# PriviligedLearningDistributedAerial/imitation

Measured on AMD Instinct MI355X. Metric: env-steps/sec (whole node) + final eval return, GAIL HalfCheetah-v4 at 1/2/4/8 MI355X, higher is better.
Workload: dtype mixed (fp32 master weights and accumulation; PPO products as split-bf16 x3 ~fp32, discriminator bf16); 1 GPU; model=GAIL: FeedForward32Policy[32,32]+RunningNorm / BasicRewardNet(32,32)+RunningNorm, global_batch=4096, seq_len=512, parallelism=dp1, engine=device, env=HalfCheetah-v4

## Files before the change

csrc/kernels/rollout.hip:

```cpp
#include <hip/hip_runtime.h>

#include "ia/engine.h"
#include "ia/envs.h"
#include "ia/wave.h"
#include "launchers.h"

namespace ia {
namespace {

constexpr int kNoiseFloats = 4096;

template <bool SPLIT>
struct Actor {
  static constexpr int KH = SPLIT ? 16 : 1;
  float w[kWaveMaxLayers][KH];
  const lf* wt[kWaveMaxLayers];
  float bias[kWaveMaxLayers];
  int k0[kWaveMaxLayers];
  int ng[kWaveMaxLayers];
  int dout[kWaveMaxLayers];
  int n_layers, hidden_act;
};

__host__ __device__ __forceinline__ int split_kh(int din) { return ((din + 1) / 2 + 3) & ~3; }
constexpr int kFullGroups = 16;
__host__ __device__ __forceinline__ int full_lds_floats(const WaveMLP& m) { return m.n_layers * 4 * kFullGroups * 64; }

__device__ __forceinline__ void nb_lane(int l, int lane, int& kh, int& ub) {
  const int r = lane >> 4;
  kh = (l & 1) ? (r >> 1) : (r & 1);
  ub = (l & 1) ? (r & 1) : (r >> 1);
}

template <bool SPLIT, bool NB = false>
__device__ void load_actor(const WaveMLP& m, Actor<SPLIT>& r, lf* wlds) {
  const int lane = threadIdx.x;
  r.n_layers = m.n_layers;
  r.hidden_act = m.hidden_act;
#pragma unroll
  for (int l = 0; l < kWaveMaxLayers; ++l) {
    int h = SPLIT ? (lane >> 5) : 0;
    int j = SPLIT ? (lane & 31) : lane;
    if (NB) {
      int ub;
      nb_lane(l, lane, h, ub);
      j = 16 * ub + (lane & 15);
    }
    const bool on = l < m.n_layers;
    const int din = on ? m.dims[l] : 0, dout = on ? m.dims[l + 1] : 0;
    const int kh = SPLIT ? split_kh(din) : 4 * kFullGroups;
    const int k0 = h ? kh : 0;
    r.k0[l] = k0;
    r.ng[l] = kh >> 2;
    r.dout[l] = dout;
    if (SPLIT) {
      const int kend = h ? din : kh;
#pragma unroll
      for (int i = 0; i < Actor<SPLIT>::KH; ++i) {
        const int k = k0 + i;
        r.w[l][i] = (on && j < dout && k < kend && k < din) ? m.W[l][j * din + k] : 0.f;
      }
    } else {
      r.wt[l] = wlds;
      if (on) {
        for (int k = 0; k < kh; ++k) wlds[((k >> 2) * 64 + lane) * 4 + (k & 3)] = (j < dout && k < din) ? m.W[l][j * din + k] : 0.f;
        wlds += kh * 64;
      }
    }
    r.bias[l] = (on && j < dout && h == 0) ? m.b[l][j] : 0.f;
  }
}

template <int HACT>
__device__ __forceinline__ float hidden_act(int act, float x) {
  if (HACT == ACT_TANH) return act_fast(ACT_TANH, x);
  if (HACT == ACT_RELU) return fmaxf(x, 0.f);
  return act_fast(act, x);
}

template <typename T>
__device__ __forceinline__ T pin(T x) {
  asm volatile("" : "+v"(x));
  return x;
}

template <bool SPLIT, int HACT, int NLT = -1, int HW = -1>
__device__ __forceinline__ float actor_forward(const Actor<SPLIT>& r, lf* xb) {
  const int lane = threadIdx.x;
  const int j = SPLIT ? (lane & 31) : lane;
  const lf4* x4 = (const lf4*)xb;
  float h = 0.f;
  const int nl = NLT > 0 ? NLT : r.n_layers;
#pragma unroll
  for (int l = 0; l < kWaveMaxLayers; ++l) {
    if (l < nl) {
      const lf4* src = x4 + (r.k0[l] >> 2);
      float acc0 = r.bias[l], acc1 = 0.f;
      if (SPLIT) {
#pragma unroll
        for (int g = 0; g < 4; ++g) {
          const f32v4 v = src[g];
          acc0 = fmaf(r.w[l][4 * g + 0], v.x, acc0);
          acc1 = fmaf(r.w[l][4 * g + 1], v.y, acc1);
          acc0 = fmaf(r.w[l][4 * g + 2], v.z, acc0);
          acc1 = fmaf(r.w[l][4 * g + 3], v.w, acc1);
        }
      } else {
        const lf4* w4 = (const lf4*)r.wt[l] + lane;
        float acc2 = 0.f, acc3 = 0.f;
#pragma unroll
        for (int g = 0; g < kFullGroups; ++g) {
          const f32v4 v = src[g], w = w4[g * 64];
          acc0 = fmaf(w.x, v.x, acc0);
          acc1 = fmaf(w.y, v.y, acc1);
          acc2 = fmaf(w.z, v.z, acc2);
          acc3 = fmaf(w.w, v.w, acc3);
        }
        acc0 += acc2;
        acc1 += acc3;
      }
      float acc = acc0 + acc1;
      if (SPLIT) acc = add_halves(acc);
      const bool last = l == nl - 1;
      const bool full = HW > 0 && !last;
      h = (full || j < r.dout[l]) ? (last ? acc : hidden_act<HACT>(r.hidden_act, acc)) : 0.f;
      if (!last) {
        wave_sync();
        if (SPLIT && HW <= 0) {
          if (lane < 32) xb[lane] = h;
        } else {
          xb[lane] = h;
        }
        wave_sync();
      }
    }
  }
  return h;
}

template <int I>
__device__ __forceinline__ float fmac_row_bcast(float acc, float x, float w) {
  if constexpr (I == 0)
    asm("s_nop 1\n\tv_fmac_f32_dpp %0, %1, %2 row_newbcast:%3 row_mask:0xf bank_mask:0xf"
        : "+v"(acc) : "v"(x), "v"(w), "i"(I));
  else
    asm("v_fmac_f32_dpp %0, %1, %2 row_newbcast:%3 row_mask:0xf bank_mask:0xf" : "+v"(acc) : "v"(x), "v"(w), "i"(I));
  return acc;
}

template <int I>
__device__ __forceinline__ void nb_dot(const float* w, float x, float& a0, float& a1) {
  if constexpr (I < 16) {
    a0 = fmac_row_bcast<I>(a0, x, w[I]);
    a1 = fmac_row_bcast<I + 1>(a1, x, w[I + 1]);
    nb_dot<I + 2>(w, x, a0, a1);
  }
}

template <int HACT, int NLT>
__device__ __forceinline__ float actor_forward_nb(const Actor<true>& r, float x) {
  static_assert(NLT > 0, "the row form needs the layer count at compile time");
#pragma unroll
  for (int l = 0; l < NLT; ++l) {
    float acc0 = r.bias[l], acc1 = 0.f;
    nb_dot<0>(r.w[l], x, acc0, acc1);
    const float acc = (l & 1) ? add_halves(acc0 + acc1) : add_rows16(acc0 + acc1);
    x = l == NLT - 1 ? acc : hidden_act<HACT>(r.hidden_act, acc);
  }
  return x;
}

__device__ __forceinline__ int actor_obs_index(int lane, int obs_dim) {
  return ((lane >> 4) & 1 ? split_kh(obs_dim) : 0) + (lane & 15);
}

__device__ __forceinline__ float env_step_lane0(const EnvParams& P, float* s, const float* action, int* term, uint64_t* rng) {
  return env_step(P, s, action, term, *rng);
}
__device__ __forceinline__ void env_reset_lane0(const EnvParams& P, float* s, float* o, uint64_t* rng) {
  env_reset(P, s, *rng);
  env_obs(P, s, o);
}

enum ChainEnv : int { CE_GENERIC = 0, CE_LOCO = 1, CE_LOCO3 = 2  };

struct LocoRegs {
  float q, qd;
  float rq[8], rv[8];
  float gear, stiff, damp, thrust, pcoup;
  float dt, drag, fwd_weight, healthy, ctrl_cost, inv_nj, inv_dt_total;
};

__device__ void loco_load(const LocoParams& p, const lf* s, LocoRegs& L) {
  const int lane = threadIdx.x, nq = loco_nq(p);
  const bool jl = lane < p.nj;
  L.q = jl ? s[p.nq_root + lane] : 0.f;
  L.qd = jl ? s[nq + p.nv_root + lane] : 0.f;
#pragma unroll
  for (int i = 0; i < 8; ++i) {
    L.rq[i] = i < p.nq_root ? s[i] : 0.f;
    L.rv[i] = i < p.nv_root ? s[nq + i] : 0.f;
  }
}

__device__ void loco_store(const LocoParams& p, const LocoRegs& L, lf* s) {
  const int lane = threadIdx.x, nq = loco_nq(p);
  if (lane < p.nj) {
    s[p.nq_root + lane] = L.q;
    s[nq + p.nv_root + lane] = L.qd;
  }
  if (lane == 0) {
#pragma unroll
    for (int i = 0; i < 8; ++i) {
      if (i < p.nq_root) s[i] = L.rq[i];
      if (i < p.nv_root) s[nq + i] = L.rv[i];
    }
  }
}

template <int ENV>
__device__ float loco_obs(const LocoParams& p, const LocoRegs& L, lf* sb, int oxi, float& ox) {
  const int lane = threadIdx.x;
  const int nr = ENV == CE_LOCO3 ? 3 : 8;
  const int nqr = ENV == CE_LOCO3 ? 3 : p.nq_root, nvr = ENV == CE_LOCO3 ? 3 : p.nv_root;
  const int npr = nqr - p.obs_skip, nj = p.nj;
  float rqi = 0.f, rvi = 0.f;
#pragma unroll
  for (int i = 0; i < nr; ++i) {
    rqi = (lane + p.obs_skip) == i ? L.rq[i] : rqi;
    rvi = lane == i ? L.rv[i] : rvi;
  }
  wave_sync();
  if (lane < npr) sb[lane] = rqi;
  if (lane < nj) {
    sb[npr + lane] = L.q;
    sb[npr + nj + nvr + lane] = L.qd;
  }
  if (lane < nvr) sb[npr + nj + lane] = rvi;
  wave_sync();
  const int D = npr + nj + nvr + nj;
  ox = sb[oxi];
  return lane < D ? sb[lane] : 0.f;
}

template <int ENV, int FS = -1>
__device__ float loco_step_regs(const LocoParams& p, LocoRegs& L, float a_in) {
  const int lane = threadIdx.x;
  const bool jl = lane < p.nj;
  const float a = jl ? fminf(fmaxf(a_in, -1.f), 1.f) : 0.f;
  const float ctrl = sum_lanes8(a * a);
  const float pitch = sum_lanes8(L.pcoup * a);
  const float x_before = L.rq[0];
  const float dt = L.dt;
  float q = L.q, qd = L.qd;
  const auto substep = [&]() {
    const float qdd = L.gear * a - L.stiff * q - L.damp * qd - 2.0f * __sinf(q);
    const float st_all = stance(q);
    const float st = jl ? st_all : 0.f;
    const float th_j = L.thrust * st * fmaxf(-qd, 0.f);
    qd = qd + dt * qdd;
    const float thrust = sum_lanes8(th_j);
    const float lift = sum_lanes8(st);
    const float vx = L.rv[0];
    L.rv[0] = vx + dt * (thrust - L.drag * vx * (1.0f + fabsf(vx)));
    if (ENV == CE_LOCO3) {
      L.rv[1] = L.rv[1] + dt * (-20.f * L.rq[1] - 4.f * L.rv[1] + 0.5f * (lift * L.inv_nj - 0.5f));
      L.rv[2] = L.rv[2] + dt * (-15.f * __sinf(L.rq[2]) - 3.f * L.rv[2] + pitch);
      L.rq[0] += dt * L.rv[0];
      L.rq[1] += dt * L.rv[1] * 1.f;
      L.rq[2] += dt * L.rv[2] * 1.f;
    } else {
      if (p.nv_root > 1) L.rv[1] = L.rv[1] + dt * (-20.f * L.rq[1] - 4.f * L.rv[1] + 0.5f * (lift * L.inv_nj - 0.5f));
      if (p.nv_root > 2) L.rv[2] = L.rv[2] + dt * (-15.f * __sinf(L.rq[2]) - 3.f * L.rv[2] + pitch);
#pragma unroll
      for (int i = 3; i < 8; ++i)
        if (i < p.nv_root) L.rv[i] = L.rv[i] * (1.f - 2.f * dt) + dt * 0.1f * pitch;
      L.rq[0] += dt * L.rv[0];
#pragma unroll
      for (int i = 1; i < 8; ++i) {
        if (i < p.nq_root) {
          if (i < p.nv_root) {
            L.rq[i] += dt * L.rv[i] * 1.f;
          } else {
            const int vi = i % p.nv_root;
            float v = 0.f;
#pragma unroll
            for (int u = 0; u < 8; ++u) v = u == vi ? L.rv[u] : v;
            L.rq[i] += dt * v * 0.1f;
          }
        }
      }
    }
    const float qn = q + dt * qd;
    const bool hi = qn > 1.2f, lo = qn < -1.2f;
    qd = (hi && qd > 0.f) || (lo && qd < 0.f) ? 0.f : qd;
    q = fminf(fmaxf(qn, -1.2f), 1.2f);
  };
  if constexpr (FS > 0) {
#pragma unroll
    for (int sub = 0; sub < FS; ++sub) substep();
  } else {
    for (int sub = 0; sub < p.frame_skip; ++sub) substep();
  }
  L.q = jl ? q : 0.f;
  L.qd = jl ? qd : 0.f;
  return L.fwd_weight * (L.rq[0] - x_before) * L.inv_dt_total + L.healthy - L.ctrl_cost * ctrl;
}

typedef __attribute__((address_space(1))) float gfl;
struct Cursors {
  gfl* obs;
  gfl* next_obs;
  gfl* act_raw;
  gfl* act_env;
  gfl* sc;
  int vec_step, act_step, sc_step;
};

__device__ __forceinline__ long long stamp(float dep) {
  long long t;
  asm volatile("s_memtime %0\n\ts_waitcnt lgkmcnt(0)" : "=s"(t) : "v"(dep));
  return t;
}

template <bool SPLIT, int ENV, int HACT, int NLT = -1, int HW = -1, int FS = -1, bool PROF = false, bool ROW = true>
__global__ __launch_bounds__(64) void rollout_chain_kernel(RolloutArgs a) {
  extern __shared__ __attribute__((aligned(16))) float lds_raw[];
  lf* xb = (lf*)lds_raw;
  lf* sb = xb + 64;
  lf* st = sb + 64;
  lf* act = st + kMaxState;
  lf* noise = act + 64;
  li* explore = (li*)(noise + kNoiseFloats);
  lf* wlds = (lf*)(explore + ((a.T + 3) & ~3));
  const int n = blockIdx.x;
  const int lane = threadIdx.x;
  const EnvParams& P = a.P;
  const int D = P.obs_dim;
  constexpr bool loco = ENV != CE_GENERIC;
  const bool discrete = !loco && a.n_actions > 0;
  const int A = discrete ? 1 : P.act_dim;
  const int AW = discrete ? a.n_actions : P.act_dim;
  const int S = state_size(P);

  constexpr bool NB = ROW && SPLIT && HW == 32 && NLT > 0;
  Actor<SPLIT> ar;
  load_actor<SPLIT, NB>(a.pi, ar, wlds);
  const int oxi = NB ? actor_obs_index(lane, D) : lane;
  const bool ox_on = oxi < D;
  const int oxr = ox_on ? oxi : lane - 64;
  const float nmean = pin((a.pi.norm_mean && ox_on) ? a.pi.norm_mean[oxi] : 0.f);
  const float nrstd = pin((a.pi.norm_mean && ox_on) ? rsqrtf(a.pi.norm_var[oxi] + a.pi.norm_eps) : 1.f);
  const float lstd = (!discrete && a.log_std && lane < A) ? a.log_std[lane] : 0.f;
  const float sd = pin(expf(lstd));
  const float lo = pin((!discrete && a.act_low && lane < A) ? a.act_low[lane] : 0.f);
  const float hi = pin((!discrete && a.act_high && lane < A) ? a.act_high[lane] : 0.f);

  for (int i = lane; i < S; i += 64) st[i] = a.state[(size_t)n * S + i];
  xb[lane] = 0.f;
  LocoRegs L{};
  if (loco) {
    const LocoParams& p = P.loco;
    const bool jl = lane < p.nj;
    L.gear = pin(jl ? p.gear[lane] : 0.f);
    L.stiff = pin(jl ? p.stiff[lane] : 0.f);
    L.damp = pin(jl ? p.damp[lane] : 0.f);
    L.thrust = pin(jl ? p.thrust[lane] : 0.f);
    L.pcoup = pin(jl ? p.pitch_coupling[lane] : 0.f);
    L.dt = pin(p.dt);
    L.drag = pin(p.drag);
    L.fwd_weight = pin(p.fwd_weight);
    L.healthy = pin(p.healthy_reward);
    L.ctrl_cost = pin(p.ctrl_cost);
    L.inv_nj = pin(1.f / (float)p.nj);
    L.inv_dt_total = pin(1.f / (p.dt * (float)p.frame_skip));
  }
  wave_sync();
  if (loco) loco_load(P.loco, st, L);

  Cursors c;
  c.vec_step = a.N * D;
  c.act_step = a.N * A;
  c.sc_step = a.N;
  c.obs = pin((gfl*)(a.obs_buf + (size_t)n * D + (lane < D ? lane : 0)));
  c.next_obs = pin((gfl*)(a.next_obs + (size_t)n * D + (lane < D ? lane : 0)));
  c.act_raw = pin((gfl*)(a.act_raw + (size_t)n * A + (lane < A ? lane : 0)));
  c.act_env = pin((gfl*)(a.act_env + (size_t)n * A + (lane < A ? lane : 0)));
  {
    float* b = lane == 0 ? a.env_rew : lane == 1 ? a.dones : lane == 2 ? a.trunc : lane == 3 ? a.ep_ret_out : a.starts;
    c.sc = pin((gfl*)(b + n));
  }

  float o = lane < D ? a.cur_obs[(size_t)n * D + lane] : 0.f;
  float ox = ox_on ? a.cur_obs[(size_t)n * D + oxi] : 0.f;
  float start = a.cur_start[n];
  uint64_t rng = a.rng[n];
  int elapsed = a.elapsed[n];
  float ep_ret = a.ep_ret[n];
  const int chunk = AW > 0 ? max(1, min(a.T, kNoiseFloats / AW)) : a.T;
  const bool has_explore = a.explore_mode != nullptr;
  const int max_steps = a.max_steps;
  long long ph[4] = {0, 0, 0, 0}, n_prof = 0;

  for (int t0 = 0; t0 < a.T; t0 += chunk) {
    const int tc = min(chunk, a.T - t0);
    wave_sync();
    for (int e = lane; e < tc * AW; e += 64) {
      const int tr = e / AW, k = e - tr * AW;
      const uint64_t key = hash3(a.seed, (uint64_t)n, (uint64_t)(a.step0 + t0 + tr));
      uint64_t s = key ^ (kLaneTweak * (uint64_t)(k + 1));
      float v;
      if (a.deterministic) {
        v = 0.f;
      } else if (discrete) {
        const float u = fmaxf(uniform01(s), 1e-12f);
        v = -logf(-logf(u));
      } else {
        v = normal01(s);
      }
      noise[e] = v;
    }
    if (has_explore)
      for (int e = lane; e < tc; e += 64) explore[e] = a.explore_mode[t0 + e];
    wave_sync();

    const lf* nz = noise + (lane < AW ? lane : 0);
    for (int tr = 0; tr < tc; ++tr, nz += AW) {
      long long t0 = 0, t1 = 0, t2 = 0, t3 = 0;
      if constexpr (PROF) t0 = stamp(o);
      if (lane < D) *c.obs = o;
      float head;
      if constexpr (NB) {
        head = actor_forward_nb<HACT, NLT>(ar, (ox - nmean) * nrstd);
      } else {
        xb[lane] = lane < D ? (o - nmean) * nrstd : 0.f;
        wave_sync();
        head = actor_forward<SPLIT, HACT, NLT, HW>(ar, xb);
      }
      float a_raw, a_env;
      if (discrete) {
        const float g = lane < a.n_actions ? head + *nz : -INFINITY;
        const float mx = wave_max(g);
        const unsigned long long m = __ballot(g == mx && lane < a.n_actions);
        const int k = m ? __builtin_ctzll(m) : a.n_actions - 1;
        a_raw = a_env = (float)k;
      } else {
        a_raw = head + sd * *nz;
        a_env = fminf(fmaxf(a_raw, lo), hi);
      }
      if (has_explore && explore[tr]) {
        const uint64_t key = hash3(a.seed, (uint64_t)n, (uint64_t)(a.step0 + t0 + tr));
        uint64_t s = key ^ kExploreTweak;
        if (discrete) {
          s ^= kExploreDiscreteTweak;
          const float u = uniform01(s);
          int k = (int)(u * (float)a.n_actions);
          k = k < a.n_actions ? k : a.n_actions - 1;
          a_raw = a_env = (float)k;
        } else {
          s ^= kLaneTweak * (uint64_t)(lane + 1);
          const float u = uniform01(s);
          a_env = lo + u * (hi - lo);
          a_raw = a_env;
        }
      }
      if (lane < A) {
        *c.act_raw = a_raw;
        *c.act_env = a_env;
      }
      int term = 0;
      float r_env;
      float o_next, ox_next;
      if constexpr (PROF) t1 = stamp(a_env);
      if (loco) {
        r_env = loco_step_regs<ENV, FS>(P.loco, L, a_env);
        if constexpr (PROF) t2 = stamp(r_env);
        o_next = loco_obs<ENV>(P.loco, L, sb, oxr, ox_next);
        if constexpr (PROF) t3 = stamp(o_next);
      } else {
        if (lane < A) act[lane] = a_env;
        wave_sync();
        if (lane == 0) {
          r_env = env_step_lane0(P, (float*)st, (const float*)act, &term, &rng);
          env_obs(P, (const float*)st, (float*)sb);
        }
        wave_sync();
        term = __builtin_amdgcn_readfirstlane(term);
        r_env = bcast(r_env, 0);
        o_next = lane < D ? sb[lane] : 0.f;
        ox_next = sb[oxr];
      }
      elapsed += 1;
      ep_ret += r_env;
      const bool trunc = !term && elapsed >= max_steps;
      const bool done = term || trunc;
      if (lane < D) *c.next_obs = o_next;
      {
        float v = start;
        v = lane == 3 ? (done ? ep_ret : 0.f) : v;
        v = lane == 2 ? (trunc ? 1.f : 0.f) : v;
        v = lane == 1 ? (done ? 1.f : 0.f) : v;
        v = lane == 0 ? r_env : v;
        if (lane < 5) *c.sc = v;
      }
      c.obs += c.vec_step;
      c.next_obs += c.vec_step;
      c.act_raw += c.act_step;
      c.act_env += c.act_step;
      c.sc += c.sc_step;
      if (done) {
        wave_sync();
        if (lane == 0) {
          if (loco) loco_reset(P.loco, (float*)st, rng);
          else env_reset_lane0(P, (float*)st, (float*)sb, &rng);
        }
        wave_sync();
        if (loco) {
          loco_load(P.loco, st, L);
          o = loco_obs<ENV>(P.loco, L, sb, oxr, ox);
        } else {
          o = lane < D ? sb[lane] : 0.f;
          ox = sb[oxr];
        }
        elapsed = 0;
        ep_ret = 0.f;
      } else {
        o = o_next;
        ox = ox_next;
      }
      start = done ? 1.f : 0.f;
      if constexpr (PROF) {
        const long long t4 = stamp(o);
        ph[0] += t1 - t0;
        ph[1] += t2 - t1;
        ph[2] += t3 - t2;
        ph[3] += t4 - t3;
        ++n_prof;
      }
    }
  }
  if constexpr (PROF) {
    if (lane < 5) a.prof[n * 5 + lane] = lane == 4 ? n_prof : lane == 0 ? ph[0] : lane == 1 ? ph[1] : lane == 2 ? ph[2] : ph[3];
  }
  if (loco) loco_store(P.loco, L, st);
  wave_sync();
  for (int i = lane; i < S; i += 64) a.state[(size_t)n * S + i] = st[i];
  if (lane < D) a.cur_obs[(size_t)n * D + lane] = o;
  if (lane == 0) {
    a.cur_start[n] = start;
    a.elapsed[n] = elapsed;
    a.ep_ret[n] = ep_ret;
  }
  rng = (uint64_t)__builtin_amdgcn_readfirstlane((int)(rng & 0xffffffffu)) |
        ((uint64_t)(unsigned)__builtin_amdgcn_readfirstlane((int)(rng >> 32)) << 32);
  if (lane == 0) a.rng[n] = rng;
}

}

bool rollout_split_form(const WaveMLP& m) {
  for (int l = 0; l <= m.n_layers; ++l)
    if (m.dims[l] > 32) return false;
  return true;
}

size_t rollout_lds_bytes(const RolloutArgs& a) {
  const size_t full = rollout_split_form(a.pi) ? 0 : (size_t)full_lds_floats(a.pi);
  return (size_t)(64 + 64 + kMaxState + 64 + kNoiseFloats + full) * sizeof(float) + (size_t)((a.T + 3) & ~3) * sizeof(int);
}

hipError_t rollout_launch(const RolloutArgs& a, hipStream_t s) {
  if (a.T <= 0 || a.N <= 0) return hipSuccess;
  if (a.P.obs_dim > 64 || a.pi.n_layers < 1 || a.pi.n_layers > kWaveMaxLayers) return hipErrorInvalidValue;
  for (int l = 0; l <= a.pi.n_layers; ++l)
    if (a.pi.dims[l] > 64 || a.pi.dims[l] < 1) return hipErrorInvalidValue;
  if (a.pi.dims[0] != a.P.obs_dim) return hipErrorInvalidValue;
  if (a.n_actions > 64 || (a.P.kind == ENV_LOCO && (a.P.loco.nj > 8 || a.n_actions > 0))) return hipErrorInvalidValue;
  const size_t lds = rollout_lds_bytes(a);
  if (lds > 160 * 1024) return hipErrorInvalidValue;
  const bool split = rollout_split_form(a.pi);
  const LocoParams& p = a.P.loco;
  const int env = a.P.kind != ENV_LOCO ? CE_GENERIC : (p.nq_root == 3 && p.nv_root == 3) ? CE_LOCO3 : CE_LOCO;
  const int act = a.pi.n_layers > 1 ? a.pi.hidden_act : ACT_IDENTITY;
  const dim3 g(a.N), b(64);
  const bool nl3 = a.pi.n_layers == 3;
  const int hw = nl3 && a.pi.dims[1] == a.pi.dims[2] ? a.pi.dims[1] : 0;
  const int fs = env == CE_LOCO3 ? p.frame_skip : 0;
  if (a.prof || a.lds_actor) {
    if (!(split && env == CE_LOCO3 && act == ACT_TANH && hw == 32 && fs == 5)) return hipErrorInvalidValue;
    if (a.prof && a.lds_actor)
      hipLaunchKernelGGL((rollout_chain_kernel<true, CE_LOCO3, ACT_TANH, 3, 32, 5, true, false>), g, b, lds, s, a);
    else if (a.prof)
      hipLaunchKernelGGL((rollout_chain_kernel<true, CE_LOCO3, ACT_TANH, 3, 32, 5, true>), g, b, lds, s, a);
    else
      hipLaunchKernelGGL((rollout_chain_kernel<true, CE_LOCO3, ACT_TANH, 3, 32, 5, false, false>), g, b, lds, s, a);
  } else if (split && env == CE_LOCO3 && act == ACT_TANH && hw == 32 && fs == 5)
    hipLaunchKernelGGL((rollout_chain_kernel<true, CE_LOCO3, ACT_TANH, 3, 32, 5>), g, b, lds, s, a);
  else if (split && env == CE_LOCO3 && act == ACT_TANH && hw == 32 && fs == 4)
    hipLaunchKernelGGL((rollout_chain_kernel<true, CE_LOCO3, ACT_TANH, 3, 32, 4>), g, b, lds, s, a);
  else if (!split && env == CE_LOCO3 && act == ACT_RELU && hw == 64 && fs == 4)
    hipLaunchKernelGGL((rollout_chain_kernel<false, CE_LOCO3, ACT_RELU, 3, 64, 4>), g, b, lds, s, a);
  else if (!split && env == CE_LOCO3 && act == ACT_RELU && hw == 64 && fs == 5)
    hipLaunchKernelGGL((rollout_chain_kernel<false, CE_LOCO3, ACT_RELU, 3, 64, 5>), g, b, lds, s, a);
  else if (split && env == CE_LOCO3 && act == ACT_TANH && hw == 32)
    hipLaunchKernelGGL((rollout_chain_kernel<true, CE_LOCO3, ACT_TANH, 3, 32>), g, b, lds, s, a);
  else if (split && env == CE_LOCO3 && act == ACT_RELU && hw == 32)
    hipLaunchKernelGGL((rollout_chain_kernel<true, CE_LOCO3, ACT_RELU, 3, 32>), g, b, lds, s, a);
  else if (!split && env == CE_LOCO3 && act == ACT_TANH && hw == 64)
    hipLaunchKernelGGL((rollout_chain_kernel<false, CE_LOCO3, ACT_TANH, 3, 64>), g, b, lds, s, a);
  else if (!split && env == CE_LOCO3 && act == ACT_RELU && hw == 64)
    hipLaunchKernelGGL((rollout_chain_kernel<false, CE_LOCO3, ACT_RELU, 3, 64>), g, b, lds, s, a);
  else if (split && env == CE_LOCO3 && act == ACT_TANH && nl3)
    hipLaunchKernelGGL((rollout_chain_kernel<true, CE_LOCO3, ACT_TANH, 3>), g, b, lds, s, a);
  else if (split && env == CE_LOCO3 && act == ACT_RELU && nl3)
    hipLaunchKernelGGL((rollout_chain_kernel<true, CE_LOCO3, ACT_RELU, 3>), g, b, lds, s, a);
  else if (!split && env == CE_LOCO3 && act == ACT_TANH && nl3)
    hipLaunchKernelGGL((rollout_chain_kernel<false, CE_LOCO3, ACT_TANH, 3>), g, b, lds, s, a);
  else if (!split && env == CE_LOCO3 && act == ACT_RELU && nl3)
    hipLaunchKernelGGL((rollout_chain_kernel<false, CE_LOCO3, ACT_RELU, 3>), g, b, lds, s, a);
  else if (split && env == CE_LOCO3 && act == ACT_TANH)
    hipLaunchKernelGGL((rollout_chain_kernel<true, CE_LOCO3, ACT_TANH>), g, b, lds, s, a);
  else if (split && env == CE_LOCO3 && act == ACT_RELU)
    hipLaunchKernelGGL((rollout_chain_kernel<true, CE_LOCO3, ACT_RELU>), g, b, lds, s, a);
  else if (!split && env == CE_LOCO3 && act == ACT_TANH)
    hipLaunchKernelGGL((rollout_chain_kernel<false, CE_LOCO3, ACT_TANH>), g, b, lds, s, a);
  else if (!split && env == CE_LOCO3 && act == ACT_RELU)
    hipLaunchKernelGGL((rollout_chain_kernel<false, CE_LOCO3, ACT_RELU>), g, b, lds, s, a);
  else if (split && env == CE_GENERIC)
    hipLaunchKernelGGL((rollout_chain_kernel<true, CE_GENERIC, -1>), g, b, lds, s, a);
  else if (!split && env == CE_GENERIC)
    hipLaunchKernelGGL((rollout_chain_kernel<false, CE_GENERIC, -1>), g, b, lds, s, a);
  else if (split)
    hipLaunchKernelGGL((rollout_chain_kernel<true, CE_LOCO, -1>), g, b, lds, s, a);
  else
    hipLaunchKernelGGL((rollout_chain_kernel<false, CE_LOCO, -1>), g, b, lds, s, a);
  return hipGetLastError();
}

}
```

Measured before the change: 1.939 million env-steps/s.

## Keep locomotion observations in registers with a lane layout matching the row-form actor

Adds a REG variant of the rollout chain kernel. Each lane is assigned the observation element that the row-broadcast actor input needs, and next observations are built with register bitmask selects instead of being staged through LDS with wave syncs. Action outputs are routed to the joint lanes with a permlane32 swap, and the first-layer DPP broadcast indices are rotated to match the new lane mapping. The goal is to remove LDS round-trips and barriers from the per-step env-to-actor critical path. The cost is more complex lane bookkeeping, and the path is gated by a host-side check that the planar locomotion layout fits.

```diff
diff --git a/csrc/kernels/rollout.hip b/csrc/kernels/rollout.hip
--- a/csrc/kernels/rollout.hip
+++ b/csrc/kernels/rollout.hip
@@ -32,8 +32,10 @@
   ub = (l & 1) ? (r & 1) : (r >> 1);
 }
 
+constexpr int kRowUnit = -2;
+
 template <bool SPLIT, bool NB = false>
-__device__ void load_actor(const WaveMLP& m, Actor<SPLIT>& r, lf* wlds) {
+__device__ void load_actor(const WaveMLP& m, Actor<SPLIT>& r, lf* wlds, int head_unit = kRowUnit) {
   const int lane = threadIdx.x;
   r.n_layers = m.n_layers;
   r.hidden_act = m.hidden_act;
@@ -45,6 +47,7 @@
       int ub;
       nb_lane(l, lane, h, ub);
       j = 16 * ub + (lane & 15);
+      if (head_unit != kRowUnit && l == m.n_layers - 1) j = head_unit < 0 ? 64 : head_unit;
     }
     const bool on = l < m.n_layers;
     const int din = on ? m.dims[l] : 0, dout = on ? m.dims[l + 1] : 0;
@@ -138,32 +141,34 @@
   return h;
 }
 
-template <int I>
+template <int I, int ROT = 0>
 __device__ __forceinline__ float fmac_row_bcast(float acc, float x, float w) {
+  constexpr int SRC = I < 8 ? ((I + 8 - ROT) & 7) : I;
   if constexpr (I == 0)
     asm("s_nop 1\n\tv_fmac_f32_dpp %0, %1, %2 row_newbcast:%3 row_mask:0xf bank_mask:0xf"
-        : "+v"(acc) : "v"(x), "v"(w), "i"(I));
+        : "+v"(acc) : "v"(x), "v"(w), "i"(SRC));
   else
-    asm("v_fmac_f32_dpp %0, %1, %2 row_newbcast:%3 row_mask:0xf bank_mask:0xf" : "+v"(acc) : "v"(x), "v"(w), "i"(I));
+    asm("v_fmac_f32_dpp %0, %1, %2 row_newbcast:%3 row_mask:0xf bank_mask:0xf" : "+v"(acc) : "v"(x), "v"(w), "i"(SRC));
   return acc;
 }
 
-template <int I>
+template <int I, int ROT = 0>
 __device__ __forceinline__ void nb_dot(const float* w, float x, float& a0, float& a1) {
   if constexpr (I < 16) {
-    a0 = fmac_row_bcast<I>(a0, x, w[I]);
-    a1 = fmac_row_bcast<I + 1>(a1, x, w[I + 1]);
-    nb_dot<I + 2>(w, x, a0, a1);
-  }
-}
-
-template <int HACT, int NLT>
+    a0 = fmac_row_bcast<I, ROT>(a0, x, w[I]);
+    a1 = fmac_row_bcast<I + 1, ROT>(a1, x, w[I + 1]);
+    nb_dot<I + 2, ROT>(w, x, a0, a1);
+  }
+}
+
+template <int HACT, int NLT, int ROT0 = 0>
 __device__ __forceinline__ float actor_forward_nb(const Actor<true>& r, float x) {
   static_assert(NLT > 0, "the row form needs the layer count at compile time");
 #pragma unroll
   for (int l = 0; l < NLT; ++l) {
     float acc0 = r.bias[l], acc1 = 0.f;
-    nb_dot<0>(r.w[l], x, acc0, acc1);
+    if (l == 0) nb_dot<0, ROT0>(r.w[l], x, acc0, acc1);
+    else nb_dot<0>(r.w[l], x, acc0, acc1);
     const float acc = (l & 1) ? add_halves(acc0 + acc1) : add_rows16(acc0 + acc1);
     x = l == NLT - 1 ? acc : hidden_act<HACT>(r.hidden_act, acc);
   }
@@ -191,11 +196,11 @@
   float dt, drag, fwd_weight, healthy, ctrl_cost, inv_nj, inv_dt_total;
 };
 
-__device__ void loco_load(const LocoParams& p, const lf* s, LocoRegs& L) {
-  const int lane = threadIdx.x, nq = loco_nq(p);
-  const bool jl = lane < p.nj;
-  L.q = jl ? s[p.nq_root + lane] : 0.f;
-  L.qd = jl ? s[nq + p.nv_root + lane] : 0.f;
+__device__ void loco_load(const LocoParams& p, const lf* s, LocoRegs& L, int jid) {
+  const int nq = loco_nq(p);
+  const bool jl = jid >= 0;
+  L.q = jl ? s[p.nq_root + jid] : 0.f;
+  L.qd = jl ? s[nq + p.nv_root + jid] : 0.f;
 #pragma unroll
   for (int i = 0; i < 8; ++i) {
     L.rq[i] = i < p.nq_root ? s[i] : 0.f;
@@ -243,10 +248,70 @@
   return lane < D ? sb[lane] : 0.f;
 }
 
+constexpr int kRegRot = 2;
+enum RegSrc : int { RS_NONE = 0, RS_Q = 1, RS_QD = 2, RS_RQ = 3 , RS_RV = 6  };
+struct RegLane {
+  int oi;
+  int src;
+  int jid;
+};
+__host__ __device__ __forceinline__ RegLane reg_lane(const LocoParams& p, int D, int lane) {
+  const int i = lane & 15, term = i < 8 ? ((i + kRegRot) & 7) : i;
+  const int oi = (((lane >> 4) & 1) ? split_kh(D) : 0) + term;
+  const int npr = 3 - p.obs_skip, nj = p.nj;
+  RegLane r{-1, RS_NONE, -1};
+  if (oi >= D) return r;
+  r.oi = oi;
+  if (oi < npr) {
+    r.src = RS_RQ + p.obs_skip + oi;
+  } else if (oi < npr + nj) {
+    r.src = RS_Q;
+    r.jid = oi - npr;
+  } else if (oi < npr + nj + 3) {
+    r.src = RS_RV + (oi - npr - nj);
+  } else {
+    r.src = RS_QD;
+    r.jid = oi - npr - nj - 3;
+  }
+  return r;
+}
+__host__ __device__ __forceinline__ int reg_head_unit(const LocoParams& p, int D, int lane) {
+  return reg_lane(p, D, (lane & 15) + (lane >= 32 ? 16 : 0)).jid;
+}
+bool reg_obs_fits(const EnvParams& P) {
+  const LocoParams& p = P.loco;
+  const int D = P.obs_dim;
+  if (P.kind != ENV_LOCO || p.nq_root != 3 || p.nv_root != 3) return false;
+  if (p.obs_skip < 0 || p.obs_skip > 2 || p.nj < 1 || p.nj > 8 || P.act_dim != p.nj) return false;
+  if (D != 3 - p.obs_skip + p.nj + 3 + p.nj || D > 32) return false;
+  if (D > 16 && split_kh(D) > 16) return false;
+  for (int i = 0; i < 8; ++i) {
+    const RegLane r = reg_lane(p, D, i);
+    if (r.jid != (i < p.nj ? i : -1) || (i < p.nj && r.src != RS_Q)) return false;
+  }
+  return true;
+}
+
+struct RegPick {
+  unsigned q, qd, rq[3], rv[3];
+};
+__device__ __forceinline__ float reg_obs(const LocoRegs& L, const RegPick& m) {
+  unsigned x = __float_as_uint(L.q) & m.q;
+  x |= __float_as_uint(L.qd) & m.qd;
+#pragma unroll
+  for (int i = 1; i < 3; ++i) x |= __float_as_uint(L.rq[i]) & m.rq[i];
+#pragma unroll
+  for (int i = 0; i < 3; ++i) x |= __float_as_uint(L.rv[i]) & m.rv[i];
+  return __uint_as_float(x);
+}
+
+__device__ __forceinline__ float reg_route(float v, bool odd_row) {
+  const auto r = __builtin_amdgcn_permlane32_swap(__float_as_uint(v), __float_as_uint(v), false, false);
+  return __uint_as_float(odd_row ? r[1] : r[0]);
+}
+
 template <int ENV, int FS = -1>
-__device__ float loco_step_regs(const LocoParams& p, LocoRegs& L, float a_in) {
-  const int lane = threadIdx.x;
-  const bool jl = lane < p.nj;
+__device__ float loco_step_regs(const LocoParams& p, LocoRegs& L, float a_in, bool jl) {
   const float a = jl ? fminf(fmaxf(a_in, -1.f), 1.f) : 0.f;
   const float ctrl = sum_lanes8(a * a);
   const float pitch = sum_lanes8(L.pcoup * a);
@@ -323,8 +388,9 @@
   return t;
 }
 
-template <bool SPLIT, int ENV, int HACT, int NLT = -1, int HW = -1, int FS = -1, bool PROF = false, bool ROW = true>
+template <bool SPLIT, int ENV, int HACT, int NLT = -1, int HW = -1, int FS = -1, bool PROF = false, bool ROW = true, bool REG = false>
 __global__ __launch_bounds__(64) void rollout_chain_kernel(RolloutArgs a) {
+  static_assert(!REG || (ROW && SPLIT && ENV == CE_LOCO3 && HW == 32 && NLT == 3), "REG: planar locomotion, row form, even head layer");
   extern __shared__ __attribute__((aligned(16))) float lds_raw[];
   lf* xb = (lf*)lds_raw;
   lf* sb = xb + 64;
@@ -345,28 +411,45 @@
 
   constexpr bool NB = ROW && SPLIT && HW == 32 && NLT > 0;
   Actor<SPLIT> ar;
-  load_actor<SPLIT, NB>(a.pi, ar, wlds);
-  const int oxi = NB ? actor_obs_index(lane, D) : lane;
+  RegLane rl{-1, RS_NONE, -1};
+  if constexpr (REG) rl = reg_lane(P.loco, D, lane);
+  const int jid = REG ? rl.jid : (loco && lane < P.loco.nj) ? lane : -1;
+  const bool jl = jid >= 0;
+  const int au = REG ? reg_head_unit(P.loco, D, lane) : lane < A ? lane : -1;
+  const bool st_on = REG ? (rl.oi >= 0 && (lane < 16 || (lane < 32 && rl.oi >= 16))) : lane < D;
+  const int sti = st_on ? (REG ? rl.oi : lane) : 0;
+  const bool odd_row = (lane >> 4) & 1;
+  load_actor<SPLIT, NB>(a.pi, ar, wlds, REG ? au : kRowUnit);
+  const int oxi = REG ? (rl.oi >= 0 ? rl.oi : D) : NB ? actor_obs_index(lane, D) : lane;
   const bool ox_on = oxi < D;
   const int oxr = ox_on ? oxi : lane - 64;
   const float nmean = pin((a.pi.norm_mean && ox_on) ? a.pi.norm_mean[oxi] : 0.f);
   const float nrstd = pin((a.pi.norm_mean && ox_on) ? rsqrtf(a.pi.norm_var[oxi] + a.pi.norm_eps) : 1.f);
-  const float lstd = (!discrete && a.log_std && lane < A) ? a.log_std[lane] : 0.f;
+  const float lstd = (!discrete && a.log_std && au >= 0) ? a.log_std[au] : 0.f;
   const float sd = pin(expf(lstd));
-  const float lo = pin((!discrete && a.act_low && lane < A) ? a.act_low[lane] : 0.f);
-  const float hi = pin((!discrete && a.act_high && lane < A) ? a.act_high[lane] : 0.f);
+  const float lo = pin((!discrete && a.act_low && au >= 0) ? a.act_low[au] : 0.f);
+  const float hi = pin((!discrete && a.act_high && au >= 0) ? a.act_high[au] : 0.f);
+  RegPick pick{};
+  if constexpr (REG) {
+    pick.q = pin(rl.src == RS_Q ? ~0u : 0u);
+    pick.qd = pin(rl.src == RS_QD ? ~0u : 0u);
+#pragma unroll
+    for (int i = 0; i < 3; ++i) {
+      pick.rq[i] = pin(rl.src == RS_RQ + i ? ~0u : 0u);
+      pick.rv[i] = pin(rl.src == RS_RV + i ? ~0u : 0u);
+    }
+  }
 
   for (int i = lane; i < S; i += 64) st[i] = a.state[(size_t)n * S + i];
   xb[lane] = 0.f;
   LocoRegs L{};
   if (loco) {
     const LocoParams& p = P.loco;
-    const bool jl = lane < p.nj;
-    L.gear = pin(jl ? p.gear[lane] : 0.f);
-    L.stiff = pin(jl ? p.stiff[lane] : 0.f);
-    L.damp = pin(jl ? p.damp[lane] : 0.f);
-    L.thrust = pin(jl ? p.thrust[lane] : 0.f);
-    L.pcoup = pin(jl ? p.pitch_coupling[lane] : 0.f);
+    L.gear = pin(jl ? p.gear[jid] : 0.f);
+    L.stiff = pin(jl ? p.stiff[jid] : 0.f);
+    L.damp = pin(jl ? p.damp[jid] : 0.f);
+    L.thrust = pin(jl ? p.thrust[jid] : 0.f);
+    L.pcoup = pin(jl ? p.pitch_coupling[jid] : 0.f);
     L.dt = pin(p.dt);
     L.drag = pin(p.drag);
     L.fwd_weight = pin(p.fwd_weight);
@@ -376,14 +459,14 @@
     L.inv_dt_total = pin(1.f / (p.dt * (float)p.frame_skip));
   }
   wave_sync();
-  if (loco) loco_load(P.loco, st, L);
+  if (loco) loco_load(P.loco, st, L, jid);
 
   Cursors c;
   c.vec_step = a.N * D;
   c.act_step = a.N * A;
   c.sc_step = a.N;
-  c.obs = pin((gfl*)(a.obs_buf + (size_t)n * D + (lane < D ? lane : 0)));
-  c.next_obs = pin((gfl*)(a.next_obs + (size_t)n * D + (lane < D ? lane : 0)));
+  c.obs = pin((gfl*)(a.obs_buf + (size_t)n * D + sti));
+  c.next_obs = pin((gfl*)(a.next_obs + (size_t)n * D + sti));
   c.act_raw = pin((gfl*)(a.act_raw + (size_t)n * A + (lane < A ? lane : 0)));
   c.act_env = pin((gfl*)(a.act_env + (size_t)n * A + (lane < A ? lane : 0)));
   {
@@ -424,14 +507,14 @@
       for (int e = lane; e < tc; e += 64) explore[e] = a.explore_mode[t0 + e];
     wave_sync();
 
-    const lf* nz = noise + (lane < AW ? lane : 0);
+    const lf* nz = noise + (REG ? (au >= 0 ? au : 0) : lane < AW ? lane : 0);
     for (int tr = 0; tr < tc; ++tr, nz += AW) {
       long long t0 = 0, t1 = 0, t2 = 0, t3 = 0;
-      if constexpr (PROF) t0 = stamp(o);
-      if (lane < D) *c.obs = o;
+      if constexpr (PROF) t0 = stamp(REG ? ox : o);
+      if (st_on) *c.obs = REG ? ox : o;
       float head;
       if constexpr (NB) {
-        head = actor_forward_nb<HACT, NLT>(ar, (ox - nmean) * nrstd);
+        head = actor_forward_nb<HACT, NLT, REG ? kRegRot : 0>(ar, (ox - nmean) * nrstd);
       } else {
         xb[lane] = lane < D ? (o - nmean) * nrstd : 0.f;
         wave_sync();
@@ -458,7 +541,7 @@
           k = k < a.n_actions ? k : a.n_actions - 1;
           a_raw = a_env = (float)k;
         } else {
-          s ^= kLaneTweak * (uint64_t)(lane + 1);
+          s ^= kLaneTweak * (uint64_t)((REG && au >= 0 ? au : lane) + 1);
           const float u = uniform01(s);
           a_env = lo + u * (hi - lo);
           a_raw = a_env;
@@ -473,9 +556,10 @@
       float o_next, ox_next;
       if constexpr (PROF) t1 = stamp(a_env);
       if (loco) {
-        r_env = loco_step_regs<ENV, FS>(P.loco, L, a_env);
+        r_env = loco_step_regs<ENV, FS>(P.loco, L, REG ? reg_route(a_env, odd_row) : a_env, jl);
         if constexpr (PROF) t2 = stamp(r_env);
-        o_next = loco_obs<ENV>(P.loco, L, sb, oxr, ox_next);
+        if constexpr (REG) o_next = ox_next = reg_obs(L, pick);
+        else o_next = loco_obs<ENV>(P.loco, L, sb, oxr, ox_next);
         if constexpr (PROF) t3 = stamp(o_next);
       } else {
         if (lane < A) act[lane] = a_env;
@@ -494,7 +578,7 @@
       ep_ret += r_env;
       const bool trunc = !term && elapsed >= max_steps;
       const bool done = term || trunc;
-      if (lane < D) *c.next_obs = o_next;
+      if (st_on) *c.next_obs = o_next;
       {
         float v = start;
         v = lane == 3 ? (done ? ep_ret : 0.f) : v;
@@ -516,8 +600,9 @@
         }
         wave_sync();
         if (loco) {
-          loco_load(P.loco, st, L);
-          o = loco_obs<ENV>(P.loco, L, sb, oxr, ox);
+          loco_load(P.loco, st, L, jid);
+          if constexpr (REG) o = ox = reg_obs(L, pick);
+          else o = loco_obs<ENV>(P.loco, L, sb, oxr, ox);
         } else {
           o = lane < D ? sb[lane] : 0.f;
           ox = sb[oxr];
@@ -545,7 +630,7 @@
   if (loco) loco_store(P.loco, L, st);
   wave_sync();
   for (int i = lane; i < S; i += 64) a.state[(size_t)n * S + i] = st[i];
-  if (lane < D) a.cur_obs[(size_t)n * D + lane] = o;
+  if (st_on) a.cur_obs[(size_t)n * D + sti] = REG ? ox : o;
   if (lane == 0) {
     a.cur_start[n] = start;
     a.elapsed[n] = elapsed;
@@ -586,15 +671,24 @@
   const bool nl3 = a.pi.n_layers == 3;
   const int hw = nl3 && a.pi.dims[1] == a.pi.dims[2] ? a.pi.dims[1] : 0;
   const int fs = env == CE_LOCO3 ? p.frame_skip : 0;
+  const bool reg = reg_obs_fits(a.P);
   if (a.prof || a.lds_actor) {
-    if (!(split && env == CE_LOCO3 && act == ACT_TANH && hw == 32 && fs == 5)) return hipErrorInvalidValue;
+    const bool fs_ok = fs == 5 || (fs == 4 && !a.prof);
+    if (!(split && env == CE_LOCO3 && act == ACT_TANH && hw == 32 && fs_ok)) return hipErrorInvalidValue;
+    if (a.prof && !a.lds_actor && !reg) return hipErrorInvalidValue;
     if (a.prof && a.lds_actor)
       hipLaunchKernelGGL((rollout_chain_kernel<true, CE_LOCO3, ACT_TANH, 3, 32, 5, true, false>), g, b, lds, s, a);
     else if (a.prof)
-      hipLaunchKernelGGL((rollout_chain_kernel<true, CE_LOCO3, ACT_TANH, 3, 32, 5, true>), g, b, lds, s, a);
+      hipLaunchKernelGGL((rollout_chain_kernel<true, CE_LOCO3, ACT_TANH, 3, 32, 5, true, true, true>), g, b, lds, s, a);
+    else if (fs == 5)
+      hipLaunchKernelGGL((rollout_chain_kernel<true, CE_LOCO3, ACT_TANH, 3, 32, 5, false, false>), g, b, lds, s, a);
     else
-      hipLaunchKernelGGL((rollout_chain_kernel<true, CE_LOCO3, ACT_TANH, 3, 32, 5, false, false>), g, b, lds, s, a);
-  } else if (split && env == CE_LOCO3 && act == ACT_TANH && hw == 32 && fs == 5)
+      hipLaunchKernelGGL((rollout_chain_kernel<true, CE_LOCO3, ACT_TANH, 3, 32, 4, false, false>), g, b, lds, s, a);
+  } else if (split && env == CE_LOCO3 && act == ACT_TANH && hw == 32 && fs == 5 && reg)
+    hipLaunchKernelGGL((rollout_chain_kernel<true, CE_LOCO3, ACT_TANH, 3, 32, 5, false, true, true>), g, b, lds, s, a);
+  else if (split && env == CE_LOCO3 && act == ACT_TANH && hw == 32 && fs == 4 && reg)
+    hipLaunchKernelGGL((rollout_chain_kernel<true, CE_LOCO3, ACT_TANH, 3, 32, 4, false, true, true>), g, b, lds, s, a);
+  else if (split && env == CE_LOCO3 && act == ACT_TANH && hw == 32 && fs == 5)
     hipLaunchKernelGGL((rollout_chain_kernel<true, CE_LOCO3, ACT_TANH, 3, 32, 5>), g, b, lds, s, a);
   else if (split && env == CE_LOCO3 && act == ACT_TANH && hw == 32 && fs == 4)
     hipLaunchKernelGGL((rollout_chain_kernel<true, CE_LOCO3, ACT_TANH, 3, 32, 4>), g, b, lds, s, a);
```

Result: no change. 1.938 million env-steps/s (-0.0%).
